# DataCTE/SDXL-Training-Improvements

Hardware: AMD Instinct MI355X
Metric: images/sec/node SDXL-base 1024^2 bf16 fwd+bwd (higher is better)
Workload: dtype bf16; 1 GPU; method=ddpm v_prediction + zero_terminal_snr + MinSNR(5), SDXL-base UNet fwd+bwd, batch 4/GPU, 1024^2 (latent 128x128); global_batch=4, parallelism=dp1, weights=synthetic (counter-hash init of the 2,567,463,684-parameter SDXL-base UNet)

## Files before the change

### sdxl-training-improvements_amd/build.py

```python
from __future__ import annotations

import os
import subprocess
import sys
from concurrent.futures import ThreadPoolExecutor
from pathlib import Path

HERE = Path(__file__).resolve().parent
CSRC = HERE / "csrc"
OBJ = HERE / "build"
LIB = HERE / "libsdxlstep.so"
OBJ_DIAG = HERE / "build_diag"
LIB_DIAG = HERE / "libsdxlstep_diag.so"
DIAG_SOURCES = ["gemm_sk.hip", "attention_pl.hip"]
SOURCES = ["gemm.hip", "gemm256.hip", "conv_wgrad3.hip", "wgrad256.hip", "gemm_cr256.hip", "gemm_pl.hip", "attention.hip", "attention_bwd_pl.hip", "norm.hip", "elementwise.hip", "loss.hip", "sampler.hip", "cond_dgrad.hip", "lora.hip", "lora_grad.hip", "optimizer.hip", "engine.hip", "capi.hip"]
HEADERS = ["common.h", "kernels.h", "gemm_tiles.h", "attn_tiles.h", "engine.h", "../../include/sdxlstep.h", "../../include/sdxlstep_diag.h"]
FLAGS = ["--offload-arch=gfx950", "-O3", "-std=c++17", "-fPIC", "-fvisibility=hidden", "-fvisibility-inlines-hidden", "-Wall", "-Wno-unused-function", "-Wno-pass-failed"]


def _hipcc() -> str:
    for c in (os.environ.get("HIPCC"), "/opt/rocm/bin/hipcc", "hipcc"):
        if c and (os.path.isabs(c) and os.path.exists(c) or not os.path.isabs(c)):
            return c
    raise RuntimeError("hipcc not found")


def _stale(target: Path, deps) -> bool:
    if not target.exists():
        return True
    t = target.stat().st_mtime
    return any(Path(d).stat().st_mtime > t for d in deps)


def build(force: bool = False, verbose: bool = True, diag: bool = False) -> Path:
    objdir, libpath = (OBJ_DIAG, LIB_DIAG) if diag else (OBJ, LIB)
    sources = SOURCES + (DIAG_SOURCES if diag else [])
    flags = FLAGS + (["-DSDXL_DIAG"] if diag else [])
    objdir.mkdir(exist_ok=True)
    hipcc = _hipcc()
    hdrs = [CSRC / h for h in HEADERS]
    jobs = []
    for s in sources:
        src, obj = CSRC / s, objdir / (s + ".o")
        if force or _stale(obj, [src] + hdrs):
            jobs.append((src, obj))

    def cc(job):
        src, obj = job
        cmd = [hipcc] + flags + ["-c", str(src), "-o", str(obj)]
        if verbose:
            print(" ".join(cmd), flush=True)
        r = subprocess.run(cmd, capture_output=True, text=True)
        if r.returncode != 0:
            raise RuntimeError(f"hipcc failed for {src.name}:\n{r.stdout}\n{r.stderr}")
        if r.stderr.strip() and verbose:
            print(r.stderr, file=sys.stderr)

    with ThreadPoolExecutor(max_workers=4) as ex:
        list(ex.map(cc, jobs))
    objs = [objdir / (s + ".o") for s in sources]
    if force or jobs or _stale(libpath, objs + [CSRC / "exports.map"]):
        cmd = [hipcc, "--offload-arch=gfx950", "-shared", "-fPIC", f"-Wl,--version-script={CSRC / 'exports.map'}", "-o", str(libpath)] + [str(o) for o in objs]
        if verbose:
            print(" ".join(cmd), flush=True)
        r = subprocess.run(cmd, capture_output=True, text=True)
        if r.returncode != 0:
            raise RuntimeError(f"link failed:\n{r.stdout}\n{r.stderr}")
    return libpath


if __name__ == "__main__":
    print(build(force="--force" in sys.argv, diag="--diag" in sys.argv))
```

### sdxl-training-improvements_amd/csrc/attention.hip

```cpp
#include "attn_tiles.h"

#include <type_traits>

#if defined(ATTN_DIAG) && (ATTN_DIAG & 256)
__device__ unsigned long long g_attn_wg[4096 * 3];
extern "C" __attribute__((visibility("default"))) int sdxl_debug_attn_wg(unsigned long long* out) {
  if (hipDeviceSynchronize() != hipSuccess) return 2;
  return hipMemcpyFromSymbol(out, HIP_SYMBOL(g_attn_wg), sizeof(unsigned long long) * 4096 * 3) == hipSuccess ? 0 : 2;
}
#endif
#if defined(ATTN_DIAG) && (ATTN_DIAG & 128)
__device__ unsigned long long g_attn_stamps[4 * 4 * 6];
extern "C" __attribute__((visibility("default"))) int sdxl_debug_attn_stamps(unsigned long long* out) {
  if (hipDeviceSynchronize() != hipSuccess) return 2;
  return hipMemcpyFromSymbol(out, HIP_SYMBOL(g_attn_stamps), sizeof(unsigned long long) * 96) == hipSuccess ? 0 : 2;
}
#endif
__global__ __launch_bounds__(256, 3) void attn_fwd_kernel(const AttnP p) {
#if defined(ATTN_DIAG) && (ATTN_DIAG & 256)
  const unsigned long long wg_t0 = __builtin_amdgcn_s_memrealtime();
#endif
  __shared__ __attribute__((aligned(16))) bf16 sm[4 * TILE_ELEMS];
  const int tid = threadIdx.x, lane = tid & 63, wave = __builtin_amdgcn_readfirstlane(tid >> 6), l16 = lane & 15, g = lane >> 4;
  int qblk, bh;
// ... 317 lines not shown
#pragma unroll
      for (int t2 = 0; t2 < 2; ++t2)
#pragma unroll
        for (int qb = 0; qb < 2; ++qb)
          dq[db][qb] = __builtin_amdgcn_mfma_f32_16x16x32_bf16(ktr[db][t2], dsf[t2][qb], dq[db][qb], 0, 0, 0);
    buf ^= 1;
  };
  const int nfull = p.Nk / 64;
  for (int t = 0; t < nfull; ++t) tile(t, std::false_type{});
  if (nfull < ntiles) tile(nfull, std::true_type{});
#pragma unroll
  for (int qb = 0; qb < 2; ++qb) {
    int q = q0 + qb * 16 + l16;
    if (q < p.Nq) {
      bf16* row = p.dQ + ((long)b * p.Nq + q) * p.lddq + h * HD;
#pragma unroll
      for (int db = 0; db < 4; ++db) {
        bf16x4 o;
        o[0] = (bf16)(dq[db][qb][0] * SCALE); o[1] = (bf16)(dq[db][qb][1] * SCALE);
        o[2] = (bf16)(dq[db][qb][2] * SCALE); o[3] = (bf16)(dq[db][qb][3] * SCALE);
        *(bf16x4*)(row + db * 16 + g * 4) = o;
      }
    }
  }
}

__global__ __launch_bounds__(256, 2) void attn_bwd_dq_kernel(const AttnP p) {
  set_wave_prio(p.prio);
  __shared__ __attribute__((aligned(16))) bf16 sm[4 * TILE_ELEMS];
  int qblk, bh;
  attn_xcd_map(p, blockIdx.x, (p.Nq + 127) >> 7, qblk, bh);
  attn_bwd_dq_body<true>(p, sm, qblk, bh);
}

template <int KB>
__device__ __forceinline__ void attn_bwd_dkv_body(const AttnP& p, bf16* sm, const int bx, const int bh, const int bz, const int nbh) {
  float (*sstat)[2][64] = (float (*)[2][64])(sm + 4 * TILE_ELEMS);
  const int tid = threadIdx.x, lane = tid & 63, wave = __builtin_amdgcn_readfirstlane(tid >> 6), l16 = lane & 15, g = lane >> 4;
  const int b = bh / p.H, h = bh - b * p.H;
  const int key0 = bx * (64 * KB) + wave * (16 * KB) + l16;
  const bf16* Qb = p.Q + (long)b * p.Nq * p.ldq + h * HD;
  const bf16* dOb = p.dO + (long)b * p.Nq * p.lddo + h * HD;
  const bf16* Kb = p.K + (long)b * p.Nk * p.ldk + h * HD;
  const bf16* Vb = p.V + (long)b * p.Nk * p.ldv + h * HD;
  bool kok[KB];
  bf16x8 kf[KB][2], vf[KB][2];
#pragma unroll
  for (int kb = 0; kb < KB; ++kb) {
    const int key = key0 + kb * 16;
    kok[kb] = key < p.Nk;
#pragma unroll
    for (int ks = 0; ks < 2; ++ks) {
      kf[kb][ks] = kok[kb] ? scale8(*(const bf16x8*)(Kb + (long)key * p.ldk + ks * 32 + g * 8), SCALE * LOG2E) : z8();
      vf[kb][ks] = kok[kb] ? *(const bf16x8*)(Vb + (long)key * p.ldv + ks * 32 + g * 8) : z8();
    }
  }
  f32x4 dk[KB][4], dv[KB][4];
#pragma unroll
  for (int kb = 0; kb < KB; ++kb)
#pragma unroll
    for (int i = 0; i < 4; ++i) { dk[kb][i] = (f32x4){0.f, 0.f, 0.f, 0.f}; dv[kb][i] = (f32x4){0.f, 0.f, 0.f, 0.f}; }

  const int ntiles_all = (p.Nq + 63) / 64;
  const int per = (ntiles_all + p.qsplit - 1) / p.qsplit;
  const int t_begin = bz * per;
  const int ntiles = min(ntiles_all, t_begin + per);
  auto load_stats = [&](int t, int bufi) {
    if (wave < 2) {
      const int q = t * 64 + lane;
      const float* src = (wave == 0 ? p.LSE : p.Delta) + (long)bh * p.Nq + q;
      lds_dma4_global(q < p.Nq ? (const void*)src : (const void*)g_attn_zero16, lds_addr_of(&sstat[bufi][wave][0]));
    }
  };
  const TileSrc qsrc = tile_src(Qb, p.ldq, wave, lane), dsrc = tile_src(dOb, p.lddo, wave, lane);
  tile_dma(qsrc, t_begin, p.Nq, sm, wave);
  tile_dma(dsrc, t_begin, p.Nq, sm + TILE_ELEMS, wave);
  load_stats(t_begin, 0);
#pragma unroll
  for (int kb = 0; kb < KB; ++kb) { landed(kf[kb][0]); landed(kf[kb][1]); landed(vf[kb][0]); landed(vf[kb][1]); }
  int buf = 0;
  auto tile = [&](int t, auto MASKC) {
    constexpr bool MASK = decltype(MASKC)::value;
    const bool more = t + 1 < ntiles;
    asm volatile("s_waitcnt vmcnt(0)" ::: "memory");
    __syncthreads();
    if (more) {
      tile_dma(qsrc, t + 1, p.Nq, sm + ((buf ^ 1) * 2) * TILE_ELEMS, wave);
      tile_dma(dsrc, t + 1, p.Nq, sm + ((buf ^ 1) * 2 + 1) * TILE_ELEMS, wave);
      load_stats(t + 1, buf ^ 1);
    }
    const bf16* Qt = sm + (buf * 2) * TILE_ELEMS;
    const bf16* Dt = Qt + TILE_ELEMS;
    bf16x8 qa[4][2], da[4][2];
#pragma unroll
    for (int qb = 0; qb < 4; ++qb) {
      qa[qb][0] = ld_frag(Qt, qb * 16 + l16, g * 8); qa[qb][1] = ld_frag(Qt, qb * 16 + l16, 32 + g * 8);
      da[qb][0] = ld_frag(Dt, qb * 16 + l16, g * 8); da[qb][1] = ld_frag(Dt, qb * 16 + l16, 32 + g * 8);
    }
    f32x4 s[KB][4], dp[KB][4];
    f32x4 ndl4[4], nl4[4];
#pragma unroll
    for (int qb = 0; qb < 4; ++qb) {
      const f32x4 dl = *(const f32x4*)&sstat[buf][1][qb * 16 + g * 4];
      const f32x4 l2 = *(const f32x4*)&sstat[buf][0][qb * 16 + g * 4];
      ndl4[qb] = (f32x4){-dl[0], -dl[1], -dl[2], -dl[3]};
      nl4[qb] = l2 * (-LOG2E);
    }
#pragma unroll
    for (int qb = 0; qb < 4; ++qb)
#pragma unroll
      for (int kb = 0; kb < KB; ++kb) {
        f32x4 a = nl4[qb];
        a = __builtin_amdgcn_mfma_f32_16x16x32_bf16(qa[qb][0], kf[kb][0], a, 0, 0, 0);
        a = __builtin_amdgcn_mfma_f32_16x16x32_bf16(qa[qb][1], kf[kb][1], a, 0, 0, 0);
        s[kb][qb] = a;
        f32x4 d = ndl4[qb];
        d = __builtin_amdgcn_mfma_f32_16x16x32_bf16(da[qb][0], vf[kb][0], d, 0, 0, 0);
        d = __builtin_amdgcn_mfma_f32_16x16x32_bf16(da[qb][1], vf[kb][1], d, 0, 0, 0);
        dp[kb][qb] = d;
      }
    bf16x8 dot[2][2], qt[2][2];
#pragma unroll
    for (int db = 0; db < 2; ++db)
#pragma unroll
      for (int t2 = 0; t2 < 2; ++t2) { dot[db][t2] = tr_frag(Dt, t2, db * 16, l16, g); qt[db][t2] = tr_frag(Qt, t2, db * 16, l16, g); }
    __builtin_amdgcn_sched_barrier(0);
    bf16x8 pf[KB][2], dsf[KB][2];
#pragma unroll
    for (int kb = 0; kb < KB; ++kb) {
      f32x4 pr[4];
#pragma unroll
      for (int qb = 0; qb < 4; ++qb) {
#pragma unroll
        for (int hh = 0; hh < 2; ++hh) {
          const f32x2 sv = (f32x2){s[kb][qb][2 * hh], s[kb][qb][2 * hh + 1]};
          f32x2 e = (f32x2){__builtin_amdgcn_exp2f(sv[0]), __builtin_amdgcn_exp2f(sv[1])};
          if (MASK) {
            if (t * 64 + qb * 16 + g * 4 + 2 * hh >= p.Nq) e[0] = 0.f;
            if (t * 64 + qb * 16 + g * 4 + 2 * hh + 1 >= p.Nq) e[1] = 0.f;
          }
          const f32x2 dpv = (f32x2){dp[kb][qb][2 * hh], dp[kb][qb][2 * hh + 1]};
          const f32x2 dsv = e * dpv;
          pr[qb][2 * hh] = e[0]; pr[qb][2 * hh + 1] = e[1];
          s[kb][qb][2 * hh] = dsv[0]; s[kb][qb][2 * hh + 1] = dsv[1];
        }
      }
      pf[kb][0] = pack8(pr[0], pr[1]);
      pf[kb][1] = pack8(pr[2], pr[3]);
      dsf[kb][0] = pack8(s[kb][0], s[kb][1]);
      dsf[kb][1] = pack8(s[kb][2], s[kb][3]);
    }
    __builtin_amdgcn_sched_barrier(0);
    bf16x8 dot2[2][2], qt2[2][2];
#pragma unroll
    for (int db = 0; db < 2; ++db)
#pragma unroll
      for (int t2 = 0; t2 < 2; ++t2) { dot2[db][t2] = tr_frag(Dt, t2, (db + 2) * 16, l16, g); qt2[db][t2] = tr_frag(Qt, t2, (db + 2) * 16, l16, g); }
#pragma unroll
    for (int db = 0; db < 2; ++db)
#pragma unroll
      for (int t2 = 0; t2 < 2; ++t2)
#pragma unroll
        for (int kb = 0; kb < KB; ++kb) {
          dv[kb][db] = __builtin_amdgcn_mfma_f32_16x16x32_bf16(dot[db][t2], pf[kb][t2], dv[kb][db], 0, 0, 0);
          dk[kb][db] = __builtin_amdgcn_mfma_f32_16x16x32_bf16(qt[db][t2], dsf[kb][t2], dk[kb][db], 0, 0, 0);
        }
    __builtin_amdgcn_sched_barrier(0);
#pragma unroll
    for (int db = 0; db < 2; ++db)
#pragma unroll
      for (int t2 = 0; t2 < 2; ++t2)
#pragma unroll
        for (int kb = 0; kb < KB; ++kb) {
          dv[kb][db + 2] = __builtin_amdgcn_mfma_f32_16x16x32_bf16(dot2[db][t2], pf[kb][t2], dv[kb][db + 2], 0, 0, 0);
          dk[kb][db + 2] = __builtin_amdgcn_mfma_f32_16x16x32_bf16(qt2[db][t2], dsf[kb][t2], dk[kb][db + 2], 0, 0, 0);
        }
    buf ^= 1;
  };
  {
    const int nfull_q = p.Nq / 64;
    for (int t = t_begin; t < ntiles; ++t) {
      if (t < nfull_q) tile(t, std::false_type{});
      else tile(t, std::true_type{});
    }
  }
#pragma unroll
  for (int kb = 0; kb < KB; ++kb) {
    const int key = key0 + kb * 16;
    if (p.qsplit > 1) {
      const int kvt = (p.Nk + 63) / 64;
      float* base = p.part + ((((long)bz * nbh + bh) * kvt * 64 + key) * 2) * 64;
#pragma unroll
      for (int db = 0; db < 4; ++db) {
        *(f32x4*)(base + db * 16 + g * 4) = dk[kb][db] * SCALE;
        *(f32x4*)(base + 64 + db * 16 + g * 4) = dv[kb][db];
      }
    } else if (kok[kb]) {
      bf16* kr = p.dK + ((long)b * p.Nk + key) * p.lddk + h * HD;
      bf16* vr = p.dV + ((long)b * p.Nk + key) * p.lddv + h * HD;
#pragma unroll
      for (int db = 0; db < 4; ++db) {
        bf16x4 a, c2;
#pragma unroll
        for (int r = 0; r < 4; ++r) { a[r] = (bf16)(dk[kb][db][r] * SCALE); c2[r] = (bf16)dv[kb][db][r]; }
        *(bf16x4*)(kr + db * 16 + g * 4) = a;
        *(bf16x4*)(vr + db * 16 + g * 4) = c2;
      }
    }
  }
}

template <int KB>
__global__ __launch_bounds__(256, 2) void attn_bwd_dkv_kernel(const AttnP p) {
  set_wave_prio(p.prio);
  __shared__ __attribute__((aligned(16))) bf16 sm[4 * TILE_ELEMS + 512];
  attn_bwd_dkv_body<KB>(p, sm, blockIdx.x, blockIdx.y, blockIdx.z, gridDim.y);
}

__global__ __launch_bounds__(256) void attn_delta_kernel(const AttnP p) {
  const long i = (long)blockIdx.x * 32 + (threadIdx.x >> 3);
  const int c = threadIdx.x & 7;
  const long total = (long)p.B * p.Nq * p.H;
  float s = 0.f;
  long bh = 0; int q = 0;
  if (i < total) {
    const int h = (int)(i % p.H);
    const long bq = i / p.H;
    q = (int)(bq % p.Nq);
    const int b = (int)(bq / p.Nq);
    bh = (long)b * p.H + h;
    const bf16x8 d = *(const bf16x8*)(p.dO + bq * p.lddo + h * HD + c * 8);
    const bf16x8 o = *(const bf16x8*)(p.O + bq * p.ldo + h * HD + c * 8);
#pragma unroll
    for (int e = 0; e < 8; ++e) s += (float)d[e] * (float)o[e];
  }
  s += __shfl_xor(s, 1, 64);
  s += __shfl_xor(s, 2, 64);
  s += __shfl_xor(s, 4, 64);
  if (i < total && c == 0) p.Delta[bh * p.Nq + q] = s;
}

template <int KB>
__global__ __launch_bounds__(256, 2) void attn_bwd_fused_kernel(const AttnP p, const int ndkv, const int nkb, const int nqb) {
  set_wave_prio(p.prio);
  __shared__ __attribute__((aligned(16))) bf16 sm[4 * TILE_ELEMS + 512];
  const int id = blockIdx.x;
  int blk, bh;
  if (id < ndkv) {
    attn_xcd_map(p, id, nkb, blk, bh);
    attn_bwd_dkv_body<KB>(p, sm, blk, bh, 0, p.B * p.H);
  } else {
    attn_xcd_map(p, id - ndkv, nqb, blk, bh);
    attn_bwd_dq_body<false>(p, sm, blk, bh);
  }
}

__global__ void attn_dkv_reduce_kernel(const AttnP p) {
  const int kvt = (p.Nk + 63) / 64;
  const long i = (long)blockIdx.x * blockDim.x + threadIdx.x;
  const long total = (long)p.B * p.H * p.Nk * 32;
  if (i >= total) return;
  const int v4 = (int)(i & 15), which = (int)((i >> 4) & 1);
  const long rk = i >> 5;
  const int key = (int)(rk % p.Nk);
  const long bh = rk / p.Nk;
  const int b = (int)(bh / p.H), h = (int)(bh - (long)b * p.H);
  f32x4 a = (f32x4){0.f, 0.f, 0.f, 0.f};
  for (int z = 0; z < p.qsplit; ++z) {
    const float* src = p.part + ((((long)z * p.B * p.H + bh) * kvt * 64 + key) * 2 + which) * 64 + v4 * 4;
    f32x4 v = *(const f32x4*)src;
    a[0] += v[0]; a[1] += v[1]; a[2] += v[2]; a[3] += v[3];
  }
  bf16x4 o;
  o[0] = (bf16)a[0]; o[1] = (bf16)a[1]; o[2] = (bf16)a[2]; o[3] = (bf16)a[3];
  bf16* dst = which == 0 ? p.dK + ((long)b * p.Nk + key) * p.lddk + h * HD : p.dV + ((long)b * p.Nk + key) * p.lddv + h * HD;
  *(bf16x4*)(dst + v4 * 4) = o;
}

size_t attn_part_floats(int B, int H, int Nk, int qsplit) {
  return qsplit > 1 ? (size_t)qsplit * B * H * ((Nk + 63) / 64) * 64 * 2 * 64 : 0;
}
int attn_pick_qsplit(int B, int H, int Nq, int Nk) {
  long blocks = (long)((Nk + 63) / 64) * B * H;
  int qt = (Nq + 63) / 64;
  int s = (int)((KNOB(36) > 0 ? KNOB(36) : 160) / blocks);
  if (s < 1) s = 1;
  if (s > qt / 2) s = qt / 2 > 0 ? qt / 2 : 1;
  if (s > 16) s = 16;
  return s;
}

static int check_attn(const AttnP& p) {
  ARG_CHECK(p.B > 0 && p.H > 0 && p.Nq > 0 && p.Nk > 0, "attention: empty problem");
  ARG_CHECK(p.ldq % 8 == 0 && p.ldk % 8 == 0 && p.ldv % 8 == 0 && p.ldo % 4 == 0,
            "attention: row strides must be multiples of 8 elements");
  return 0;
}

int launch_attn_fwd(const AttnP& p, hipStream_t st) {
  if (int e = check_attn(p)) return e;
#ifdef SDXL_DIAG
  if (KNOB(33) == 2 && attn_fwd_pl_applicable(p)) return launch_attn_fwd_pl(p, st);
#endif
  return launch_attn_fwd_tiled(p, st);
}
int launch_attn_fwd_tiled(const AttnP& p, hipStream_t st) {
  if (int e = check_attn(p)) return e;
  if (FILE* f = launch_log()) { fprintf(f, "A,0,%d,%d,%d,%d\n", p.B, p.H, p.Nq, p.Nk); fflush(f); }
  AttnP q = p;
  q.xcd = (p.B * p.H) % 8 == 0 && KNOB(32) != 1;
  hipLaunchKernelGGL(attn_fwd_kernel, dim3(cdiv(p.Nq, 128) * p.B * p.H), dim3(256), 0, st, q);
  HIP_CHECK_RET(hipGetLastError());
  return 0;
}

static int check_attn_bwd(const AttnP& p) {
  if (int e = check_attn(p)) return e;
  ARG_CHECK(p.O && p.dO && p.dQ && p.dK && p.dV && p.LSE && p.Delta, "attention bwd: missing buffers");
  ARG_CHECK(!p.accumulate, "attention bwd: accumulate not implemented");
  return 0;
}
int launch_attn_bwd_dq(const AttnP& p, hipStream_t st) {
  if (int e = check_attn_bwd(p)) return e;
  if (FILE* f = launch_log()) { fprintf(f, "A,1,%d,%d,%d,%d\n", p.B, p.H, p.Nq, p.Nk); fflush(f); }
  AttnP q = p;
  q.xcd = (p.B * p.H) % 8 == 0 && KNOB(32) != 1;
  hipLaunchKernelGGL(attn_bwd_dq_kernel, dim3(cdiv(p.Nq, 128) * p.B * p.H), dim3(256), 0, st, q);
  HIP_CHECK_RET(hipGetLastError());
  return 0;
}
int launch_attn_bwd_dkv(const AttnP& p, hipStream_t st) {
  if (int e = check_attn_bwd(p)) return e;
  if (FILE* f = launch_log()) { fprintf(f, "A,2,%d,%d,%d,%d\n", p.B, p.H, p.Nq, p.Nk); fflush(f); }
  AttnP q = p;
  if (q.qsplit < 1 || !q.part) q.qsplit = 1;
  if (q.qsplit == 1 && (long)cdiv(p.Nk, 128) * p.B * p.H >= 1024)
    hipLaunchKernelGGL(attn_bwd_dkv_kernel<2>, dim3(cdiv(p.Nk, 128), p.B * p.H, 1), dim3(256), 0, st, q);
  else
    hipLaunchKernelGGL(attn_bwd_dkv_kernel<1>, dim3(cdiv(p.Nk, 64), p.B * p.H, q.qsplit), dim3(256), 0, st, q);
  if (q.qsplit > 1) {
    long total = (long)p.B * p.H * p.Nk * 32;
    hipLaunchKernelGGL(attn_dkv_reduce_kernel, dim3(cdiv(total, 256)), dim3(256), 0, st, q);
  }
  HIP_CHECK_RET(hipGetLastError());
  return 0;
}
int launch_attn_bwd_fused(const AttnP& p, hipStream_t st) {
  if (int e = check_attn_bwd(p)) return e;
  ARG_CHECK(p.lddo % 8 == 0 && p.ldo % 8 == 0, "attention bwd (fused): dO / O row strides must be multiples of 8 elements");
  if (FILE* f = launch_log()) { fprintf(f, "A,1,%d,%d,%d,%d\nA,2,%d,%d,%d,%d\n", p.B, p.H, p.Nq, p.Nk, p.B, p.H, p.Nq, p.Nk); fflush(f); }
  AttnP q = p;
  q.qsplit = 1;
  q.xcd = (p.B * p.H) % 8 == 0 && KNOB(32) != 1;
  const long total = (long)p.B * p.Nq * p.H;
  if (!p.delta_ready) hipLaunchKernelGGL(attn_delta_kernel, dim3(cdiv(total, 32)), dim3(256), 0, st, q);
  if (KNOB(35) != 1 && ((p.Nq >= 2048 && p.Nk >= 2048) || KNOB(35) == 2) && attn_bwd_pl_applicable(q)) return launch_attn_bwd_pl(q, st);
  const int nkb = cdiv(p.Nk, 128), nqb = cdiv(p.Nq, 128), nbh = p.B * p.H;
  hipLaunchKernelGGL(attn_bwd_fused_kernel<2>, dim3(nkb * nbh + nqb * nbh), dim3(256), 0, st, q, nkb * nbh, nkb, nqb);
  HIP_CHECK_RET(hipGetLastError());
  return 0;
}
int launch_attn_bwd(const AttnP& p, hipStream_t st) {
  const bool fused = (KNOB(20) != 1 || p.delta_ready) && (p.qsplit <= 1 || !p.part) && p.Nk >= 256 && p.lddo % 8 == 0 && p.ldo % 8 == 0;
  if (fused) return launch_attn_bwd_fused(p, st);
  if (int e = launch_attn_bwd_dq(p, st)) return e;
  return launch_attn_bwd_dkv(p, st);
}
```

### sdxl-training-improvements_amd/csrc/kernels.h

```cpp
#pragma once
#include "common.h"

#define SDXL_NKNOBS 40
#ifdef SDXL_DIAG
extern int g_knobs[SDXL_NKNOBS];
#define KNOB(i) (g_knobs[(i)])
constexpr bool SDXL_DIAG_BUILD = true;
constexpr bool SDXL_UP2_3 = true;
constexpr bool SDXL_LN_EPILOGUE = true;
#else
#define KNOB(i) 0
constexpr bool SDXL_DIAG_BUILD = false;
constexpr bool SDXL_UP2_3 = false;
constexpr bool SDXL_LN_EPILOGUE = false;
#endif

enum { GEMM_NT = 0, GEMM_NN = 1, GEMM_TN = 2 };
#define GEMM_LAUNCH(kernel, grid, block, smem, st, p)                                                          \
  do {                                                                                                         \
    if ((p).anyorder) hipExtLaunchKernelGGL(kernel, grid, block, smem, st, nullptr, nullptr, hipExtAnyOrderLaunch, p); \
    else hipLaunchKernelGGL(kernel, grid, block, smem, st, p);                                                 \
  } while (0)

#define GEMM_MAX_GROUP 4
struct GemmP {
  int form;
  const bf16* A;
  const bf16* B;
  void* C;
  int M, N, K;
  long lda, ldb, ldc;
  int taps;
  int Hm, Wm, Hs, Ws, sm, sd;
  int flip;
  int up2;
  int up_plane, up_rows;
  long b_tap_stride;
  long c_tap_stride;
  const bf16* bias;
  const bf16* resid;
  long ldr;
  const bf16* rowvec;
  long ldv;
  int rows_per_batch;
  int geglu;
  int geglu_group;
  bf16* aux;
  long ldaux;
  int out_f32;
  int accumulate;
  int splitk;
  float* slab;
  long slab_ld;
  bf16* Cb;
  float cb_scale;
  float* bias_grad;
  const bf16* delta_o;
  long delta_ldo;
  float* delta_out;
  int delta_nq, delta_heads;
  const bf16* ln_x;
  long ln_ldx;
  const float* ln_stats;
  const bf16* ln_gamma;
  bf16* ln_dx;
  const bf16* ln_addend;
  long ln_ldo;
  float* ln_part;
  int ln_epoch;
  float* ln_pcol;
  int xcd_px;
  int xcd_bh;
  int tail_n0;
  int anyorder;
  int cfg;
  int prio;
  int group;
  const bf16* gA[GEMM_MAX_GROUP];
  const bf16* gB[GEMM_MAX_GROUP];
  float* gC[GEMM_MAX_GROUP];
  float* gbias_grad[GEMM_MAX_GROUP];
  bf16* gCb[GEMM_MAX_GROUP];
};

__device__ __forceinline__ void gemm_bias_out(float* bias_grad, float* slab, long slab_ld, int splitk, int split, int M, int m, float v) {
  if (splitk > 1) slab[(long)splitk * M * slab_ld + (long)split * M + m] = v;
  else atomicAdd(bias_grad + m, v);
}
int gemm_pick_group(int M, int N, int taps, long red, int splitk);
size_t gemm_slab_floats(int M, int N, int taps, int splitk);
void gemm_defaults(GemmP* p);
int launch_gemm(const GemmP& p, hipStream_t st);
enum { GEMM_K128 = 0, GEMM_K256, GEMM_KCR256, GEMM_KPL, GEMM_KWGRAD256, GEMM_KCONV_WGRAD3, GEMM_KSK };
enum { GEMM_POST_NONE = 0, GEMM_POST_REDUCE, GEMM_POST_EPILOGUE };
struct GemmRoute {
  int kernel;
  int cfg;
  bool fast;
  int post;
};
GemmRoute gemm_route(const GemmP& p);
int gemm_route_checked(GemmP p, GemmRoute* r);
bool gemm256_applicable(const GemmP& p);
void gemm_set_mode(int mode);
bool gemm_use256(int form, int M, int N, int K, int splitk);
int gemm_pick_splitk(int M, int N, int taps, long red);
int gemm_pick_splitk_small(int M, int N, int K, int kind = -1);
int linear_wgrad_splitk(int Mo, int No, long rows);
int conv3x3_fwd_splitk(int B, int H, int W, int Cin, int Cout, int stride);
int conv3x3_dgrad_splitk(int B, int H, int W, int Cin, int Cout, int stride);
int conv3x3_wgrad_splitk(int B, int H, int W, int Cin, int Cout, int stride);
int upconv3x3_fwd_splitk(int B, int H, int W, int Cin, int Cout);
int upconv3x3_dgrad_splitk(int B, int H, int W, int Cin, int Cout);
GemmP conv3x3_fwd_problem(int B, int H, int W, int Cin, int Cout, int stride);
GemmP conv3x3_dgrad_problem(int B, int H, int W, int Cin, int Cout, int stride);
GemmP conv3x3_wgrad_problem(int B, int H, int W, int Cin, int Cout, int stride);
int launch_gemm256(const GemmP& p, hipStream_t st);
void gemm256_set_tail(bool on);
#ifdef SDXL_DIAG
bool gemm_sk_applicable(const GemmP& p);
int launch_gemm_sk(const GemmP* problems, int n, hipStream_t st);
int launch_gemm_multi(const GemmP* problems, int n, hipStream_t st);
void gemm_set_sk_mode(int mode);
int gemm_sk_mode();
bool gemm_use_sk(const GemmP& p);
void gemm_sk_set_workers(int n);
int gemm_ln_error(unsigned* out);
int gemm_sk_error(hipStream_t st, unsigned* out);
#endif
bool conv_wgrad3_applicable(const GemmP& p);
bool conv_wgrad3_policy(int M, int N, long red, int Wm, int stride);
int conv_wgrad3_pick_splitk(int M, int N, long red);
int launch_conv_wgrad3(const GemmP& p, hipStream_t st);
void conv_wgrad3_set_enabled(bool on);
bool wgrad256_applicable(const GemmP& p);
bool wgrad256_policy(int M, int N, long red);
int wgrad256_pick_splitk(int M, int N, long red);
int launch_wgrad256(const GemmP& p, hipStream_t st);
void wgrad256_set_enabled(bool on);
bool cr256_applicable(const GemmP& p);
int launch_cr256(const GemmP& p, int bn, hipStream_t st, bool deep = false, bool phased = false);
int cr256_wgrad_cfg(int M, int N, long red, bool bias);
bool pl_applicable(const GemmP& p);
int launch_pl(const GemmP& p, int bn, hipStream_t st, bool prefetch = false);
int launch_pl_prefetch_b(const GemmP& p, int parts, hipStream_t st);
int gemm_ln_cfg(int M, int N, int K);
size_t gemm_ln_part_floats(int M, int N);
size_t gemm_ln_pcol_floats(int M, int N);
int gemm_ln_rowblocks(int M);
int cr256_pick_splitk(int M, int N, long red, int cfg);
int gemm_profile_begin();
FILE* launch_log();
bool gemm_profiling();
int gemm_profile_end(double* flops, double* ms, int* launches);

struct AttnP {
  const bf16 *Q, *K, *V;
  bf16* O;
  float* LSE;
  int B, H, Nq, Nk;
  long ldq, ldk, ldv, ldo;
  const bf16* dO;
  long lddo;
  bf16 *dQ, *dK, *dV;
  long lddq, lddk, lddv;
  float* Delta;
  int accumulate;
  int qsplit;
  float* part;
  int prio;
  int delta_ready;
  int xcd;
};
size_t attn_part_floats(int B, int H, int Nk, int qsplit);
int attn_pick_qsplit(int B, int H, int Nq, int Nk);
int launch_attn_fwd(const AttnP& p, hipStream_t st);
int launch_attn_fwd_tiled(const AttnP& p, hipStream_t st);
bool attn_fwd_pl_applicable(const AttnP& p);
int launch_attn_fwd_pl(const AttnP& p, hipStream_t st);
bool attn_bwd_pl_applicable(const AttnP& p);
int launch_attn_bwd_pl(const AttnP& p, hipStream_t st);
int launch_attn_bwd(const AttnP& p, hipStream_t st);
int launch_attn_bwd_dq(const AttnP& p, hipStream_t st);
int launch_attn_bwd_dkv(const AttnP& p, hipStream_t st);
int launch_attn_bwd_fused(const AttnP& p, hipStream_t st);

size_t groupnorm_ws_floats(int B, int C, int G);
int launch_groupnorm_fwd(const bf16* x, bf16* y, const bf16* gamma, const bf16* beta, float* stats,
                         float* ws, int B, int HW, int C, int G, float eps, int silu,
                         hipStream_t st);
int launch_groupnorm_bwd(const bf16* x, const bf16* dy, const bf16* gamma, const bf16* beta,
                         const float* stats, bf16* dx, const bf16* addend, float* dgamma, float* dbeta, float* ws,
                         int B, int HW, int C, int G, int silu, hipStream_t st, float* prow = nullptr);
int launch_layernorm_fwd(const bf16* x, bf16* y, const bf16* gamma, const bf16* beta, float* stats, int M,
                         int C, float eps, hipStream_t st);
size_t layernorm_bwd_part_floats(int M, int C);
int launch_layernorm_bwd(const bf16* x, const bf16* dy, const bf16* gamma, const float* stats, bf16* dx,
                         const bf16* addend, float* part, int* nblk_out, int M, int C, hipStream_t st);
int launch_layernorm_param_grads(const bf16* x, const bf16* dy, const float* stats, float* dgamma, float* dbeta, int M, int C, hipStream_t st);
int layernorm_param_partial_rows(int M, int C);
int launch_layernorm_param_partials(const bf16* x, const bf16* dy, const float* stats, float* part, int M, int C, hipStream_t st);
#define LN_RED_MAX 64
struct LnRedEntry { const float* part; float* dgamma; float* dbeta; int nblk, C; };
struct LnRedBatch { LnRedEntry e[LN_RED_MAX]; int n; };
int launch_ln_param_reduce(const LnRedBatch& b, hipStream_t st);

int launch_silu_fwd(const bf16* x, bf16* y, long n, hipStream_t st);
int launch_silu_bwd(const bf16* x, const bf16* dy, bf16* dx, const bf16* addend, long n, hipStream_t st);
int launch_add(const bf16* a, const bf16* b, bf16* o, long n, hipStream_t st);
size_t colsum_part_floats(int batches, int rows, int N);
int launch_colsum_f32_batched(const bf16* x, float* out, int batches, int rows, int N, long ldx, long ld_out, float* part, hipStream_t st);
int launch_colsum_partials(const bf16* x, float* out, int batches, int rows, int N, long ldx, long ld_out, float* part, LnRedEntry* entries, hipStream_t st);
int launch_concat(const bf16* a, int Ca, const bf16* b, int Cb, bf16* o, long rows, hipStream_t st);
int launch_split_add(const bf16* g, bf16* ga, int Ca, const bf16* add_a, bf16* gb, int Cb, const bf16* add_b,
                     long rows, hipStream_t st);
int launch_upsample2x(const bf16* x, bf16* y, int B, int H, int W, int C, hipStream_t st);
int launch_upconv_fold_weights(const bf16* w, bf16* weff, int Cout, int Cin, hipStream_t st);
int launch_pixel_shuffle2(const bf16* src, bf16* dst, int B, int H, int W, int C, int to_hi, hipStream_t st, const bf16* addend = nullptr);
static inline long upconv_plane_rows(int B, int H, int W) { return ((long)B * H * W + 127) / 128 * 128; }
int launch_upconv3x3_fwd(const bf16* x, const bf16* w, const bf16* bias, bf16* weff, bf16* planar, bf16* y, int B, int H, int W, int Cin,
                         int Cout, int splitk, float* slab, hipStream_t st);
#ifdef SDXL_DIAG
int launch_conv3x3_s2_fwd(const bf16* x, const bf16* w, const bf16* bias, bf16* xplanar, bf16* y, int B, int H, int W, int Cin, int Cout,
                          hipStream_t st);
int launch_conv3x3_s2_wgrad(const bf16* dy, const bf16* xplanar, float* dw, float* dbias, bf16* emit, float emit_scale, int accumulate, int B,
                            int H, int W, int Cin, int Cout, int splitk, float* slab, hipStream_t st);
#endif
int launch_conv3x3_s2_dgrad(const bf16* dy, const bf16* w, bf16* planar, bf16* dx, const bf16* addend, int B, int H, int W, int Cin,
                            int Cout, int prio, hipStream_t st);
int launch_upconv_unfold_grads(const float* dweff, float* dw, bf16* emit, float emit_scale, int accumulate, int Cout, int Cin, hipStream_t st);
int launch_upconv3x3_wgrad(const bf16* planar, const bf16* x, float* dweff, float* dw, float* dbias, bf16* emit, float emit_scale,
                           int accumulate, int B, int H, int W, int Cin, int Cout, int splitk, float* slab, hipStream_t st);
int launch_upconv3x3_dgrad(const bf16* dy, const bf16* weff, bf16* planar, bf16* dx, const bf16* addend, int B, int H, int W, int Cin,
                           int Cout, int splitk, float* slab, int prio, hipStream_t st);
int launch_upsample2x_bwd(const bf16* dy, bf16* dx, const bf16* addend, int B, int H, int W, int C, hipStream_t st);
int launch_sincos(const float* t, bf16* out, int rows, int dim, long ldo, hipStream_t st);
int launch_copy_cols(const bf16* src, long lds, bf16* dst, long ldd, int rows, int cols, hipStream_t st);
int launch_f32_to_bf16(const float* x, bf16* y, long n, float scale, hipStream_t st);
int launch_bf16_to_f32(const bf16* x, float* y, long n, hipStream_t st);
int launch_sumsq_f32(const float* x, long n, float* out , hipStream_t st);
int launch_sumsq_bf16(const bf16* x, long n, float* out , hipStream_t st);
int launch_clip_coef(const float* sumsq, float max_norm, float* coef, hipStream_t st);
int launch_scale_f32(float* x, long n, const float* scale_dev, hipStream_t st);
int launch_exchange_shadow(void* buf, size_t bytes, int workgroups, int lds_bytes, float busy_us, hipStream_t st);

struct LossP {
  int method;
  int prediction_type;
  int use_min_snr;
  float min_snr_gamma;
  int use_ztsnr;
  int B, HW, C;
  const float* latents;
  const float* noise;
  const float* sigma;
  const float* tag_w;
  bf16* unet_in;
  const bf16* pred;
  bf16* dpred;
  float grad_scale;
  float* out;
  float* part;
  int loss_type;
  float huber_c;
  const float* sample_w;
  const float* huber_cb;
  float* ps_out;
  const float* noise_in;
  const float* mask;
  int mask_norm;
  float* mnorm;
};
static inline __host__ __device__ int loss_ps_slots(int B, int HW) { const int s = 255 / HW + 2; return s < B ? s : B; }
static inline size_t loss_part_floats(int B, int HW) { return (6 + 2 * (size_t)loss_ps_slots(B, HW)) * (((size_t)B * HW + 255) / 256); }
int launch_loss_prepare(const LossP& p, hipStream_t st);
int launch_loss_fwd(const LossP& p, hipStream_t st);
int launch_loss_bwd(const LossP& p, hipStream_t st);

struct SamplerP {
  float* x;
  const bf16* pred;
  bf16* x_in;
  int B, HW;
  int cfg, init;
  float a_skip, a_out, p, q, a_in_next, clamp, guidance, rescale;
  float* part;
  int ext;
  float* hist;
  float* xsave;
  const float* noise;
  float r, u, s;
  int save;
  const float* mask;
  const float* known;
  const float* knoise;
  float k_a, k_b;
};
static inline size_t sampler_part_floats(int B, int HW) { return 4 * (size_t)B * (((size_t)HW + 255) / 256); }
int launch_sampler_step(const SamplerP& p, hipStream_t st);

struct OptimP {
  bf16* p;
  const float* grad_f32;
  const bf16* grad_bf16;
  bf16 *m, *v;
  size_t n;
  float beta1, beta2;
  float one_minus_beta2;
  float eps_bf16;
  int grad_round_bf16;
  const float* grad_scale;
  float* ema;
  float ema_omd;
};
struct AdamWP : OptimP {
  bf16* shift;
  float one_minus_beta1;
  float value;
  float decay_alpha_bf16;
  int reference_ema;
  const unsigned short* rand;
  unsigned seed_lo, seed_hi, step_counter;
  size_t elem_offset;
};
int launch_adamw_bf16(const AdamWP& q, hipStream_t st);
struct SfkP : OptimP {
  bf16* c;
  float one_minus_beta1_bf16;
  int has_wd;
  float wd_alpha_bf16;
  float neg_step;
  float step;
  float decay;
};
int launch_sfk(const SfkP& q, int reference, hipStream_t st);
int launch_adamw_decay(bf16* shift, const bf16* p, size_t n, float alpha_bf16, hipStream_t st);


struct CondDgradP {
  int n;
  const bf16* A[2];
  const bf16* W[2];
  long lda[2], ldb[2];
  int K[2];
  float* C;
  long ldc;
  int M, N;
  float* slab;
  const float* gate;
};
size_t cond_dgrad_slab_floats(int n, const int* K, int M, int N);
int launch_cond_dgrad(const CondDgradP& p, hipStream_t st);

#define LORA_M_ROWS 32
#define LORA_M_COLS 64
#define LORA_M_KC 32
#define LORA_B_ROWS 32
#define LORA_B_COLS 256
#define LORA_B_KC 16
#define LORA_A_COLS 128
#define LORA_A_ROWS 32
struct LoraTarget {
  long w_off;
  long base_off;
  long a_off, b_off;
  long ga_off, gb_off;
  int out, in;
  int tile_m, tile_b, tile_a;
  int kind;
  int cg;
  int nrows;
};
#define LORA_KIND_PLAIN 0
#define LORA_KIND_CONV3 1
#define LORA_KIND_GEGLU 2
__host__ __device__ static inline int lora_src_col(int kind, int cg, int j) {
  return kind == LORA_KIND_CONV3 ? (j % cg) * 9 + j / cg : j;
}
__host__ __device__ static inline int lora_src_row(int kind, int cg, int c4, int r) {
  if (kind != LORA_KIND_GEGLU) return r;
  const int grp = r / (2 * cg), rem = r - grp * 2 * cg, half = rem / cg;
  return half * c4 + grp * cg + rem - half * cg;
}
struct LoraP {
  const LoraTarget* table;
  LoraTarget one;
  int n, rank;
  float scale;
  int tiles_m, tiles_b, tiles_a;
  int mapped;
  bf16* w;
  const bf16* base;
  const bf16 *a, *b;
  const float* dw;
  float *ga, *gb;
};
static inline int lora_tiles_m(int out, int in) { return cdiv(out, LORA_M_ROWS) * cdiv(in, LORA_M_COLS); }
static inline int lora_tiles_b(int out, int in) { return cdiv(out, LORA_B_ROWS); }
static inline int lora_tiles_a(int out, int in) { return cdiv(in, LORA_A_COLS); }
int launch_lora_merge(const LoraP& p, hipStream_t st);
int launch_lora_project(const LoraP& p, hipStream_t st);

#define LORA_G_CHUNK 512
struct LoraGradTarget {
  long a_off, b_off;
  long ga_off, gb_off;
  long part_off;
  int out, in;
  int dy_col;
  int tile0, red0;
  int pad;
};
struct LoraGradP {
  const LoraGradTarget* table;
  LoraGradTarget one;
  int n, rank;
  float scale;
  int accumulate;
  const bf16* x; long ldx;
  const bf16* dy; long ldy;
  int M, Mp;
  int xvec, yvec;
  int nchunk, tiles, reds;
  const bf16 *a, *b;
  float *ga, *gb;
  bf16* tu;
  float* part;
};
static inline int lora_grad_rb(int rank) { return rank <= 16 ? 1 : rank <= 32 ? 2 : rank <= 64 ? 4 : 8; }
static inline int lora_grad_mp(int M) { return cdiv(M, 64) * 64; }
static inline int lora_grad_chunks(int M) { return cdiv(M, LORA_G_CHUNK); }
static inline size_t lora_grad_tu_elems(int n, int rank, int M) { return (size_t)n * 2 * 16 * lora_grad_rb(rank) * lora_grad_mp(M); }
static inline size_t lora_grad_part_floats(int out, int in, int rank, int M) { return (size_t)lora_grad_chunks(M) * rank * ((size_t)in + out); }
static inline int lora_grad_tiles(int out, int in) { return cdiv(in, 128) + cdiv(out, 128); }
static inline int lora_grad_reds(int out, int in, int rank) { return cdiv((long)rank * ((long)in + out), 256); }
int launch_lora_grad(const LoraGradP& p, hipStream_t st);
```

Before: 37.22 images/sec.

## Add short-key attention kernels for cross-attention forward and dQ backward

Adds specialized attention kernels for problems with at most 80 keys, which covers SDXL cross-attention over 77 text tokens. K and V are staged once per block into registers, and the block loops over several query tiles with a single-pass softmax instead of online rescaling. The launch grid is sized to the number of available slots. These kernels are meant to cut the repeated K/V loads and the flash-loop overhead that the general tiled kernel pays on short key sequences. The backward dQ kernel also computes Delta inline, which has to agree with what the dK/dV kernel expects.

```diff
diff --git a/sdxl-training-improvements_amd/build.py b/sdxl-training-improvements_amd/build.py
--- a/sdxl-training-improvements_amd/build.py
+++ b/sdxl-training-improvements_amd/build.py
@@ -13,7 +13,7 @@
 OBJ_DIAG = HERE / "build_diag"
 LIB_DIAG = HERE / "libsdxlstep_diag.so"
 DIAG_SOURCES = ["gemm_sk.hip", "attention_pl.hip"]
-SOURCES = ["gemm.hip", "gemm256.hip", "conv_wgrad3.hip", "wgrad256.hip", "gemm_cr256.hip", "gemm_pl.hip", "attention.hip", "attention_bwd_pl.hip", "norm.hip", "elementwise.hip", "loss.hip", "sampler.hip", "cond_dgrad.hip", "lora.hip", "lora_grad.hip", "optimizer.hip", "engine.hip", "capi.hip"]
+SOURCES = ["gemm.hip", "gemm256.hip", "conv_wgrad3.hip", "wgrad256.hip", "gemm_cr256.hip", "gemm_pl.hip", "attention.hip", "attention_sk.hip", "attention_bwd_pl.hip", "norm.hip", "elementwise.hip", "loss.hip", "sampler.hip", "cond_dgrad.hip", "lora.hip", "lora_grad.hip", "optimizer.hip", "engine.hip", "capi.hip"]
 HEADERS = ["common.h", "kernels.h", "gemm_tiles.h", "attn_tiles.h", "engine.h", "../../include/sdxlstep.h", "../../include/sdxlstep_diag.h"]
 FLAGS = ["--offload-arch=gfx950", "-O3", "-std=c++17", "-fPIC", "-fvisibility=hidden", "-fvisibility-inlines-hidden", "-Wall", "-Wno-unused-function", "-Wno-pass-failed"]
 
diff --git a/sdxl-training-improvements_amd/csrc/attention.hip b/sdxl-training-improvements_amd/csrc/attention.hip
--- a/sdxl-training-improvements_amd/csrc/attention.hip
+++ b/sdxl-training-improvements_amd/csrc/attention.hip
@@ -643,6 +643,7 @@
 #ifdef SDXL_DIAG
   if (KNOB(33) == 2 && attn_fwd_pl_applicable(p)) return launch_attn_fwd_pl(p, st);
 #endif
+  if (KNOB(40) != 1 && attn_sk_applicable(p)) return launch_attn_sk_fwd(p, st);
   return launch_attn_fwd_tiled(p, st);
 }
 int launch_attn_fwd_tiled(const AttnP& p, hipStream_t st) {
@@ -663,6 +664,7 @@
 }
 int launch_attn_bwd_dq(const AttnP& p, hipStream_t st) {
   if (int e = check_attn_bwd(p)) return e;
+  if (KNOB(40) != 1 && attn_sk_dq_applicable(p)) return launch_attn_sk_bwd_dq(p, st);
   if (FILE* f = launch_log()) { fprintf(f, "A,1,%d,%d,%d,%d\n", p.B, p.H, p.Nq, p.Nk); fflush(f); }
   AttnP q = p;
   q.xcd = (p.B * p.H) % 8 == 0 && KNOB(32) != 1;
diff --git a/sdxl-training-improvements_amd/csrc/attention_sk.hip b/sdxl-training-improvements_amd/csrc/attention_sk.hip
--- /dev/null
+++ b/sdxl-training-improvements_amd/csrc/attention_sk.hip
@@ -0,0 +1,266 @@
+#include "attn_tiles.h"
+
+#define SK_KEYS 80
+#define SK_KB 5
+
+__device__ __forceinline__ s16x4 sk_tr_half(const bf16* tile, int row0, int col0, int l16, int g) {
+  const int r = row0 + g * 4 + (l16 >> 2);
+  const int v = (col0 >> 3) + ((l16 >> 1) & 1);
+  return __builtin_amdgcn_ds_read_tr16_b64_v4i16((lds_s16x4*)(tile + r * 64 + ((v ^ (r & 7)) << 3) + (l16 & 1) * 4));
+}
+__device__ __forceinline__ void sk_stage(const bf16* src, long ld, int nk, bf16* tile, int tid) {
+  bf16x8 x[3];
+#pragma unroll
+  for (int i = 0; i < 3; ++i) {
+    const int idx = tid + i * 256, r = idx >> 3, v = idx & 7;
+    x[i] = r < nk && idx < SK_KEYS * 8 ? *(const bf16x8*)(src + (long)r * ld + v * 8) : z8();
+  }
+#pragma unroll
+  for (int i = 0; i < 3; ++i) {
+    const int idx = tid + i * 256, r = idx >> 3, v = idx & 7;
+    if (idx < SK_KEYS * 8) *(bf16x8*)(tile + r * 64 + ((v ^ (r & 7)) << 3)) = x[i];
+  }
+}
+__device__ __forceinline__ void sk_row_frags(const bf16* tile, int l16, int g, bf16x8 (&f)[SK_KB][2]) {
+#pragma unroll
+  for (int kb = 0; kb < SK_KB; ++kb) {
+    f[kb][0] = ld_frag(tile, kb * 16 + l16, g * 8);
+    f[kb][1] = ld_frag(tile, kb * 16 + l16, 32 + g * 8);
+  }
+}
+__device__ __forceinline__ void sk_tr_frags(const bf16* tile, int l16, int g, bf16x8 (&f)[4][3]) {
+#pragma unroll
+  for (int db = 0; db < 4; ++db) {
+    f[db][0] = tr_frag(tile, 0, db * 16, l16, g);
+    f[db][1] = tr_frag(tile, 1, db * 16, l16, g);
+    union { s16x4 s[2]; bf16x8 v; } u;
+    u.s[0] = sk_tr_half(tile, 64, db * 16, l16, g);
+    u.s[1] = (s16x4){0, 0, 0, 0};
+    f[db][2] = u.v;
+  }
+}
+__device__ __forceinline__ void sk_second_product(const bf16x8 (&f)[4][3], const f32x4 (&s)[SK_KB], f32x4 (&out)[4]) {
+  const bf16x8 b0 = pack8(s[0], s[1]), b1 = pack8(s[2], s[3]), b2 = pack8(s[4], (f32x4){0.f, 0.f, 0.f, 0.f});
+#pragma unroll
+  for (int db = 0; db < 4; ++db) {
+    f32x4 a = (f32x4){0.f, 0.f, 0.f, 0.f};
+    a = __builtin_amdgcn_mfma_f32_16x16x32_bf16(f[db][0], b0, a, 0, 0, 0);
+    a = __builtin_amdgcn_mfma_f32_16x16x32_bf16(f[db][1], b1, a, 0, 0, 0);
+    out[db] = __builtin_amdgcn_mfma_f32_16x16x32_bf16(f[db][2], b2, a, 0, 0, 0);
+  }
+}
+
+__global__ __launch_bounds__(256, 3) void attn_sk_fwd_kernel(const AttnP p, const int nchunk, const int per) {
+  __shared__ __attribute__((aligned(16))) bf16 sm[2 * SK_KEYS * 64];
+  const int tid = threadIdx.x, lane = tid & 63, wave = __builtin_amdgcn_readfirstlane(tid >> 6), l16 = lane & 15, g = lane >> 4;
+  int chunk, bh;
+  attn_xcd_map(p, blockIdx.x, nchunk, chunk, bh);
+  const int b = bh / p.H, h = bh - b * p.H;
+  const bf16* Qb = p.Q + (long)b * p.Nq * p.ldq + h * HD;
+  const bf16* Kb = p.K + (long)b * p.Nk * p.ldk + h * HD;
+  const bf16* Vb = p.V + (long)b * p.Nk * p.ldv + h * HD;
+  const int u_end = min((p.Nq + 127) >> 7, (chunk + 1) * per);
+  int u = chunk * per;
+
+  auto load_q = [&](int uu, bf16x8 (&qf)[2][2]) {
+#pragma unroll
+    for (int qb = 0; qb < 2; ++qb) {
+      const int q = uu * 128 + wave * 32 + qb * 16 + l16;
+#pragma unroll
+      for (int ks = 0; ks < 2; ++ks) qf[qb][ks] = q < p.Nq ? *(const bf16x8*)(Qb + (long)q * p.ldq + ks * 32 + g * 8) : z8();
+    }
+  };
+  bf16x8 qn[2][2];
+  load_q(u, qn);
+  sk_stage(Kb, p.ldk, p.Nk, sm, tid);
+  sk_stage(Vb, p.ldv, p.Nk, sm + SK_KEYS * 64, tid);
+  __syncthreads();
+  bf16x8 kf[SK_KB][2];
+  sk_row_frags(sm, l16, g, kf);
+  bf16x8 vt[4][3];
+  sk_tr_frags(sm + SK_KEYS * 64, l16, g, vt);
+
+  for (; u < u_end; ++u) {
+    bf16x8 qf[2][2];
+#pragma unroll
+    for (int qb = 0; qb < 2; ++qb) { qf[qb][0] = qn[qb][0]; qf[qb][1] = qn[qb][1]; }
+    if (u + 1 < u_end) load_q(u + 1, qn);
+    const int q0 = u * 128 + wave * 32;
+    if (q0 >= p.Nq) continue;
+#pragma unroll
+    for (int qb = 0; qb < 2; ++qb) {
+      f32x4 st[SK_KB];
+#pragma unroll
+      for (int kb = 0; kb < SK_KB; ++kb) {
+        f32x4 a = (f32x4){0.f, 0.f, 0.f, 0.f};
+        a = __builtin_amdgcn_mfma_f32_16x16x32_bf16(kf[kb][0], qf[qb][0], a, 0, 0, 0);
+        st[kb] = __builtin_amdgcn_mfma_f32_16x16x32_bf16(kf[kb][1], qf[qb][1], a, 0, 0, 0);
+      }
+#pragma unroll
+      for (int kb = 0; kb < SK_KB; ++kb)
+        if ((kb + 1) * 16 > p.Nk) {
+#pragma unroll
+          for (int r = 0; r < 4; ++r)
+            if (kb * 16 + g * 4 + r >= p.Nk) st[kb][r] = -1e30f;
+        }
+      float mx = st[0][0];
+#pragma unroll
+      for (int kb = 0; kb < SK_KB; ++kb)
+#pragma unroll
+        for (int r = 0; r < 4; ++r) mx = fmaxf(mx, st[kb][r]);
+      mx = max_over_g(mx);
+      const f32x2 c2 = (f32x2){SCALE * LOG2E, SCALE * LOG2E}, m2 = (f32x2){-mx * (SCALE * LOG2E), -mx * (SCALE * LOG2E)};
+      f32x2 ls2 = (f32x2){0.f, 0.f};
+#pragma unroll
+      for (int kb = 0; kb < SK_KB; ++kb)
+#pragma unroll
+        for (int hh = 0; hh < 2; ++hh) {
+          const f32x2 arg = (f32x2){st[kb][2 * hh], st[kb][2 * hh + 1]} * c2 + m2;
+          const f32x2 e = (f32x2){__builtin_amdgcn_exp2f(arg[0]), __builtin_amdgcn_exp2f(arg[1])};
+          st[kb][2 * hh] = e[0]; st[kb][2 * hh + 1] = e[1];
+          ls2 += e;
+        }
+      const float l = sum_over_g(ls2[0] + ls2[1]);
+      f32x4 ot[4];
+      sk_second_product(vt, st, ot);
+      const float inv = 1.f / l;
+      const int q = q0 + qb * 16 + l16;
+      if (q < p.Nq) {
+        bf16* orow = p.O + ((long)b * p.Nq + q) * p.ldo + h * HD;
+#pragma unroll
+        for (int db = 0; db < 4; ++db) {
+          bf16x4 o;
+          o[0] = (bf16)(ot[db][0] * inv); o[1] = (bf16)(ot[db][1] * inv); o[2] = (bf16)(ot[db][2] * inv); o[3] = (bf16)(ot[db][3] * inv);
+          *(bf16x4*)(orow + db * 16 + g * 4) = o;
+        }
+        if (g == 0 && p.LSE) p.LSE[(long)bh * p.Nq + q] = mx * SCALE + __builtin_amdgcn_logf(l) * (1.f / LOG2E);
+      }
+    }
+  }
+}
+
+__global__ __launch_bounds__(256, 2) void attn_sk_bwd_dq_kernel(const AttnP p, const int nchunk, const int per) {
+  set_wave_prio(p.prio);
+  __shared__ __attribute__((aligned(16))) bf16 sm[2 * SK_KEYS * 64];
+  const int tid = threadIdx.x, lane = tid & 63, wave = __builtin_amdgcn_readfirstlane(tid >> 6), l16 = lane & 15, g = lane >> 4;
+  int chunk, bh;
+  attn_xcd_map(p, blockIdx.x, nchunk, chunk, bh);
+  const int b = bh / p.H, h = bh - b * p.H;
+  const bf16* Qb = p.Q + (long)b * p.Nq * p.ldq + h * HD;
+  const bf16* dOb = p.dO + (long)b * p.Nq * p.lddo + h * HD;
+  const bf16* Ob = p.O + (long)b * p.Nq * p.ldo + h * HD;
+  const bf16* Kb = p.K + (long)b * p.Nk * p.ldk + h * HD;
+  const bf16* Vb = p.V + (long)b * p.Nk * p.ldv + h * HD;
+  const int u_end = min((p.Nq + 63) >> 6, (chunk + 1) * per);
+  int u = chunk * per;
+
+  struct Rows { bf16x8 q[2], d[2], o[2]; float lse; };
+  auto load_rows = [&](int uu, Rows& r) {
+    const int q = uu * 64 + wave * 16 + l16;
+    const bool ok = q < p.Nq;
+#pragma unroll
+    for (int ks = 0; ks < 2; ++ks) {
+      r.q[ks] = ok ? *(const bf16x8*)(Qb + (long)q * p.ldq + ks * 32 + g * 8) : z8();
+      r.d[ks] = ok ? *(const bf16x8*)(dOb + (long)q * p.lddo + ks * 32 + g * 8) : z8();
+      r.o[ks] = ok ? *(const bf16x8*)(Ob + (long)q * p.ldo + ks * 32 + g * 8) : z8();
+    }
+    r.lse = ok ? p.LSE[(long)bh * p.Nq + q] : 0.f;
+  };
+  Rows rn;
+  load_rows(u, rn);
+  sk_stage(Kb, p.ldk, p.Nk, sm, tid);
+  sk_stage(Vb, p.ldv, p.Nk, sm + SK_KEYS * 64, tid);
+  __syncthreads();
+  bf16x8 kf[SK_KB][2], vf[SK_KB][2];
+  sk_row_frags(sm, l16, g, kf);
+  sk_row_frags(sm + SK_KEYS * 64, l16, g, vf);
+  bf16x8 kt[4][3];
+  sk_tr_frags(sm, l16, g, kt);
+
+  for (; u < u_end; ++u) {
+    const Rows r = rn;
+    if (u + 1 < u_end) load_rows(u + 1, rn);
+    const int q = u * 64 + wave * 16 + l16;
+    if (u * 64 + wave * 16 >= p.Nq) continue;
+    float dl = 0.f;
+#pragma unroll
+    for (int ks = 0; ks < 2; ++ks)
+#pragma unroll
+      for (int e = 0; e < 8; ++e) dl += (float)r.d[ks][e] * (float)r.o[ks][e];
+    dl = sum_over_g(dl);
+    if (q < p.Nq && g == 0) p.Delta[(long)bh * p.Nq + q] = dl;
+    const f32x2 c2 = (f32x2){SCALE * LOG2E, SCALE * LOG2E}, nl2 = (f32x2){-r.lse * LOG2E, -r.lse * LOG2E};
+    f32x4 st[SK_KB], dp[SK_KB];
+#pragma unroll
+    for (int kb = 0; kb < SK_KB; ++kb) {
+      f32x4 a = (f32x4){0.f, 0.f, 0.f, 0.f};
+      a = __builtin_amdgcn_mfma_f32_16x16x32_bf16(kf[kb][0], r.q[0], a, 0, 0, 0);
+      st[kb] = __builtin_amdgcn_mfma_f32_16x16x32_bf16(kf[kb][1], r.q[1], a, 0, 0, 0);
+      f32x4 d = (f32x4){-dl, -dl, -dl, -dl};
+      d = __builtin_amdgcn_mfma_f32_16x16x32_bf16(vf[kb][0], r.d[0], d, 0, 0, 0);
+      dp[kb] = __builtin_amdgcn_mfma_f32_16x16x32_bf16(vf[kb][1], r.d[1], d, 0, 0, 0);
+    }
+#pragma unroll
+    for (int kb = 0; kb < SK_KB; ++kb) {
+#pragma unroll
+      for (int hh = 0; hh < 2; ++hh) {
+        const f32x2 arg = (f32x2){st[kb][2 * hh], st[kb][2 * hh + 1]} * c2 + nl2;
+        const f32x2 pr = (f32x2){__builtin_amdgcn_exp2f(arg[0]), __builtin_amdgcn_exp2f(arg[1])};
+        const f32x2 ds = pr * (f32x2){dp[kb][2 * hh], dp[kb][2 * hh + 1]};
+        st[kb][2 * hh] = ds[0]; st[kb][2 * hh + 1] = ds[1];
+      }
+      if ((kb + 1) * 16 > p.Nk) {
+#pragma unroll
+        for (int rr = 0; rr < 4; ++rr)
+          if (kb * 16 + g * 4 + rr >= p.Nk) st[kb][rr] = 0.f;
+      }
+    }
+    f32x4 dq[4];
+    sk_second_product(kt, st, dq);
+    if (q < p.Nq) {
+      bf16* row = p.dQ + ((long)b * p.Nq + q) * p.lddq + h * HD;
+#pragma unroll
+      for (int db = 0; db < 4; ++db) {
+        bf16x4 o;
+        o[0] = (bf16)(dq[db][0] * SCALE); o[1] = (bf16)(dq[db][1] * SCALE); o[2] = (bf16)(dq[db][2] * SCALE); o[3] = (bf16)(dq[db][3] * SCALE);
+        *(bf16x4*)(row + db * 16 + g * 4) = o;
+      }
+    }
+  }
+}
+
+static void sk_grid(int nunits, int nbh, int slots, int& nchunk, int& per) {
+  int cmax = slots * cdiv(nbh, slots) / nbh;
+  if (cmax > nunits) cmax = nunits;
+  per = cdiv(nunits, cmax);
+  if (KNOB(40) >= 16) per = KNOB(40) - 16 < nunits ? KNOB(40) - 16 : nunits;
+  nchunk = cdiv(nunits, per);
+}
+
+bool attn_sk_applicable(const AttnP& p) {
+  return p.Nk >= 1 && p.Nk <= SK_KEYS && p.ldq % 8 == 0 && p.ldk % 8 == 0 && p.ldv % 8 == 0 && p.ldo % 4 == 0 && (long)p.B * p.H < (1 << 20) &&
+         ((size_t)p.Q | (size_t)p.K | (size_t)p.V) % 16 == 0 && (size_t)p.O % 8 == 0;
+}
+bool attn_sk_dq_applicable(const AttnP& p) {
+  return attn_sk_applicable(p) && p.lddo % 8 == 0 && p.ldo % 8 == 0 && p.lddq % 4 == 0 && ((size_t)p.dO | (size_t)p.O) % 16 == 0 && (size_t)p.dQ % 8 == 0;
+}
+int launch_attn_sk_fwd(const AttnP& p, hipStream_t st) {
+  if (FILE* f = launch_log()) { fprintf(f, "AS,0,%d,%d,%d,%d\n", p.B, p.H, p.Nq, p.Nk); fflush(f); }
+  AttnP q = p;
+  q.xcd = (p.B * p.H) % 8 == 0 && KNOB(32) != 1;
+  int nchunk, per;
+  sk_grid(cdiv(p.Nq, 128), p.B * p.H, 768, nchunk, per);
+  hipLaunchKernelGGL(attn_sk_fwd_kernel, dim3(nchunk * p.B * p.H), dim3(256), 0, st, q, nchunk, per);
+  HIP_CHECK_RET(hipGetLastError());
+  return 0;
+}
+int launch_attn_sk_bwd_dq(const AttnP& p, hipStream_t st) {
+  if (FILE* f = launch_log()) { fprintf(f, "AS,1,%d,%d,%d,%d\n", p.B, p.H, p.Nq, p.Nk); fflush(f); }
+  AttnP q = p;
+  q.xcd = (p.B * p.H) % 8 == 0 && KNOB(32) != 1;
+  int nchunk, per;
+  sk_grid(cdiv(p.Nq, 64), p.B * p.H, 512, nchunk, per);
+  hipLaunchKernelGGL(attn_sk_bwd_dq_kernel, dim3(nchunk * p.B * p.H), dim3(256), 0, st, q, nchunk, per);
+  HIP_CHECK_RET(hipGetLastError());
+  return 0;
+}
diff --git a/sdxl-training-improvements_amd/csrc/kernels.h b/sdxl-training-improvements_amd/csrc/kernels.h
--- a/sdxl-training-improvements_amd/csrc/kernels.h
+++ b/sdxl-training-improvements_amd/csrc/kernels.h
@@ -1,7 +1,7 @@
 #pragma once
 #include "common.h"
 
-#define SDXL_NKNOBS 40
+#define SDXL_NKNOBS 41
 #ifdef SDXL_DIAG
 extern int g_knobs[SDXL_NKNOBS];
 #define KNOB(i) (g_knobs[(i)])
@@ -180,6 +180,10 @@
 int launch_attn_fwd_pl(const AttnP& p, hipStream_t st);
 bool attn_bwd_pl_applicable(const AttnP& p);
 int launch_attn_bwd_pl(const AttnP& p, hipStream_t st);
+bool attn_sk_applicable(const AttnP& p);
+bool attn_sk_dq_applicable(const AttnP& p);
+int launch_attn_sk_fwd(const AttnP& p, hipStream_t st);
+int launch_attn_sk_bwd_dq(const AttnP& p, hipStream_t st);
 int launch_attn_bwd(const AttnP& p, hipStream_t st);
 int launch_attn_bwd_dq(const AttnP& p, hipStream_t st);
 int launch_attn_bwd_dkv(const AttnP& p, hipStream_t st);
```

Result: no change. 37.16 images/sec (-0.2%).
